# hassony2/homan

Measured on AMD Instinct MI355X. Metric: optimisation iters/sec (30-frame 256^2 clip), higher is better.
Workload: dtype f32

## Files before the change

### homan_amd/csrc/raster_lines.hip

```cpp
#include "raster_ws.h"

__global__ __launch_bounds__(256) void k_bwd_masks(const float* __restrict__ gin, int mode,
                                                   const float* __restrict__ upstream,
                                                   const float* __restrict__ keep_sum, int B, int S,
                                                   const unsigned short* __restrict__ alpha16,
                                                   float* __restrict__ gimg, unsigned short* __restrict__ planes,
                                                   int clip_len)
{
    if (mode == 1 && upstream[0] > 0.0f) return;
    const int w = threadIdx.x >> 6, lane = threadIdx.x & 63;
    const int is = 2 * S, tiles_x = S / HM_TILE, ntiles = tiles_x * tiles_x;
    const int tile = blockIdx.x * 4 + w, b = blockIdx.y;
    if (tile >= ntiles) return;
    const int ty = tile / tiles_x, tx = tile % tiles_x;
    const int rr = lane >> 3, cc = lane & 7;
    const int r = ty * HM_TILE + rr, c = tx * HM_TILE + cc;
    const long po = ((long)b * S + r) * S + c;
    unsigned long long cq[4];
#pragma unroll
    for (int dy = 0; dy < 2; ++dy) {
        const unsigned aw = alpha16[(((long)b * (is / 16) + ty) * (is / 16) + tx) * 16 + 2 * rr + dy];
#pragma unroll
        for (int dx = 0; dx < 2; ++dx) cq[2 * dy + dx] = __ballot((aw >> (2 * cc + dx)) & 1u);
    }
    unsigned long long nq[4], pq[4];
    if (mode == 3) {
#pragma unroll
        for (int dy = 0; dy < 2; ++dy) {
            const long at = ((long)b * is + 2 * r + dy) * is + 2 * c;
            const float2 g2 = *reinterpret_cast<const float2*>(gin + at);
            *reinterpret_cast<float2*>(gimg + at) = g2;
            nq[2 * dy] = __ballot(g2.x < 0.0f); pq[2 * dy] = __ballot(g2.x > 0.0f);
            nq[2 * dy + 1] = __ballot(g2.y < 0.0f); pq[2 * dy + 1] = __ballot(g2.y > 0.0f);
        }
    } else {
        float g = gin[po];
        if (mode == 1) {
            float s = upstream[0] * 2.0f;
            g = s * g / keep_sum[b / clip_len] / (float)clip_len;
        }
        gimg[po] = g;
        const unsigned long long nb1 = __ballot(g < 0.0f), pb1 = __ballot(g > 0.0f);
#pragma unroll
        for (int k = 0; k < 4; ++k) { nq[k] = nb1; pq[k] = pb1; }
    }
    const Ballots4 cov = {cq[0], cq[1], cq[2], cq[3]}, nbv = {nq[0], nq[1], nq[2], nq[3]}, pbv = {pq[0], pq[1], pq[2], pq[3]};
    emit_planes(cov, nbv, pbv, b, B, is, tx, ty, lane, planes);
}


__device__ __forceinline__ int sweep_family(float a0, float a1, int is, int& d0_from)
{
    d0_from = 0;
    if (!(a0 != a1)) return 0;
    d0_from = (int)fmaxf(ceilf(fminf(a0, a1)), 0.0f);
    const int d0_to = (int)fminf(fmaxf(a0, a1), (float)is - 1.0f);
    return max(0, d0_to - d0_from + 1);
}

__device__ __forceinline__ int sweep_face_record(long bf, const float* __restrict__ faces9, const FaceBox* __restrict__ boxes,
                                                 const unsigned char* __restrict__ owned, int F, int is, SweepFace& rec)
{
    const int b = (int)(bf / F), fi = (int)(bf - (long)b * F);
    const unsigned mask = (reinterpret_cast<const uint2*>(boxes)[bf].x >> 14) & 3u;
    const unsigned char own0 = owned[(long)b * 2 * F + fi], own1 = owned[(long)b * 2 * F + F + fi];
    const float* src = faces9 + bf * 9;
    float sx[3], sy[3];
#pragma unroll
    for (int k = 0; k < 3; ++k) { sx[k] = src[3 * k]; sy[k] = src[3 * k + 1]; }
    const bool act0 = (mask & 1u) && own0;
    const bool act1 = (mask & 2u) && own1;
    if (!(act0 || act1)) return 0;
#pragma unroll
    for (int k = 0; k < 3; ++k) { rec.px[k] = topix(sx[k], is); rec.py[k] = topix(sy[k], is); }
    int n = 0;
#pragma unroll
    for (int var = 0; var < 2; ++var)
#pragma unroll
        for (int e = 0; e < 3; ++e)
#pragma unroll
            for (int axis = 0; axis < 2; ++axis) {
                const int k0 = e, k1 = (e + 1) % 3;
                const int v0 = var ? 2 - k0 : k0, v1 = var ? 2 - k1 : k1;
                int from;
                const int c = sweep_family(axis ? rec.py[v0] : rec.px[v0], axis ? rec.py[v1] : rec.px[v1], is, from);
                if (var ? act1 : act0) n += c;
                rec.cum[var * 6 + e * 2 + axis] = (unsigned short)n;
            }
    rec.bf = (int)bf;
    rec.b = b;
    return n;
}

__device__ __forceinline__ void sweep_compact(int blk, int nblk, int fpt, const float* __restrict__ faces9,
                                              const FaceBox* __restrict__ boxes, const unsigned char* __restrict__ owned,
                                              int B, int F, int is, double* __restrict__ parts, const SweepList& sl,
                                              int clip_len)
{
    __shared__ int s_wsum[4][2];
    __shared__ unsigned long long s_base;
    const int tid = threadIdx.x, lane = tid & 63, wv = tid >> 6;
    const int per_clip = nblk / (B / clip_len), clip = blk / per_clip;
    const long cbase = (long)clip * clip_len * F;
    const long bf0 = cbase + ((long)(blk - clip * per_clip) * 256 + tid) * fpt, nbf = cbase + (long)clip_len * F;
    int nk[4], n = 0, hasf = 0;
#pragma unroll
    for (int k = 0; k < 4; ++k) {
        SweepFace rec;
        nk[k] = (k < fpt && bf0 + k < nbf) ? sweep_face_record(bf0 + k, faces9, boxes, owned, F, is, rec) : 0;
        n += nk[k];
        hasf += nk[k] > 0 ? 1 : 0;
    }
    const int inc_i = hm_wave_scan_incl(n), inc_f = hm_wave_scan_incl(hasf);
    if (lane == 63) { s_wsum[wv][0] = inc_i; s_wsum[wv][1] = inc_f; }
    __syncthreads();
    int pre_i = 0, pre_f = 0, tot_i = 0, tot_f = 0;
#pragma unroll
    for (int k = 0; k < 4; ++k) {
        if (k < wv) { pre_i += s_wsum[k][0]; pre_f += s_wsum[k][1]; }
        tot_i += s_wsum[k][0];
        tot_f += s_wsum[k][1];
    }
    if (tid == 0)
        s_base = tot_f ? atomicAdd(sl.cnt, ((unsigned long long)tot_f << 32) | (unsigned)((tot_i + SWEEP_UNIT - 1) & ~(SWEEP_UNIT - 1))) : 0ull;
    __syncthreads();
    const unsigned long long base = s_base;
    int off = (int)(base & 0xffffffffull) + pre_i + inc_i - n;
    int idx = (int)(base >> 32) + pre_f + inc_f - hasf;
#pragma unroll
    for (int k = 0; k < 4; ++k) {
        const long bf = bf0 + k;
        if (k >= fpt || bf >= nbf) break;
        bool zero = nk[k] == 0;
        if (nk[k] > 0) {
            SweepFace rec;
            const int nn = sweep_face_record(bf, faces9, boxes, owned, F, is, rec);
            const int u_lo = off >> SWEEP_USHIFT, u_hi = (off + nn - 1) >> SWEEP_USHIFT;
            const bool over = u_hi >= sl.ucap || u_hi + idx >= sl.slot_cap;
            rec.off = off;
            rec.flags = over ? 1 : 0;
            zero = u_hi > u_lo;
            const uint4* r4 = reinterpret_cast<const uint4*>(&rec);
            uint4* t4 = reinterpret_cast<uint4*>(sl.tab + idx);
#pragma unroll
            for (int q = 0; q < 4; ++q) t4[q] = r4[q];
            sl.offs[idx] = off;
            for (int u = (off + SWEEP_UNIT - 1) >> SWEEP_USHIFT; (u << SWEEP_USHIFT) < off + nn && u < sl.ucap; ++u)
                sl.ufirst[u] = (unsigned)idx;
            off += nn;
            ++idx;
        }
        if (zero) {
            double* o = parts + bf * 6;
#pragma unroll
            for (int q = 0; q < 6; ++q) o[q] = 0.0;
        }
    }
    if (tid == 0) {
        const unsigned int t = atomicAdd(sl.done, 1u);
        if (t == (unsigned)nblk - 1u) {
            sl.total[0] = atomicExch(sl.cnt, 0ull);
            atomicExch(sl.done, 0u);
        }
    }
}


#ifndef LINES_NL
#define LINES_NL 2
#endif
#ifdef LINES_REVERSED
#define LINES_BLK(i, n) ((n) - 1 - (i))
#else
#define LINES_BLK(i, n) (i)
#endif
template <bool W32>
__global__ __launch_bounds__(256) void k_bwd_lines(const unsigned short* __restrict__ planes,
                                                   const float* __restrict__ gimg, const float* __restrict__ dimg,
                                                   int mode, const float* __restrict__ upstream,
                                                   const float* __restrict__ keep_sum,
                                                   const int* __restrict__ idx_map, int B, int S,
                                                   SweepSrc* __restrict__ srcs, uint4* __restrict__ lrec,
                                                   int ncomp, int fpt, const float* __restrict__ faces9,
                                                   const FaceBox* __restrict__ boxes,
                                                   const unsigned char* __restrict__ owned, int F,
                                                   double* __restrict__ parts, SweepList sl, int clip_len,
                                                   unsigned short* __restrict__ lsum, int nred,
                                                   const float* __restrict__ red_partials, float* __restrict__ frame_rec,
                                                   float* __restrict__ loss_out, int out_stride,
                                                   const unsigned int* __restrict__ ts_flag,
                                                   unsigned long long* __restrict__ ts_slots)
{
    HM_CHAIN_KERNEL();
    const unsigned long long ts_t0 = (unsigned long long)wall_clock64();
    const bool ts_on = hm_ts_enabled(ts_flag) && threadIdx.x == 0;
    if (ts_on) hm_ts_store(ts_slots, blockIdx.x, 0, ts_t0);
    const int blk = (int)blockIdx.x;
    __shared__ unsigned long long s_w[16][LINES_NL][SWEEP_CUMW];
    __shared__ int s_ex[16][LINES_NL][SWEEP_CUMW];
    if (blk < ncomp) {
        sweep_compact(blk, ncomp, fpt, faces9, boxes, owned, B, F, 2 * S, parts, sl, clip_len);
        if (ts_on) hm_ts_store(ts_slots, blockIdx.x, 1, (unsigned long long)wall_clock64());
        return;
    }
    if (blk < ncomp + nred) {
        sil_reduce_frame(blk - ncomp, red_partials, (S / 8) * (S / 8), keep_sum, frame_rec, loss_out, nullptr, clip_len,
                         out_stride);
        if (ts_on) hm_ts_store(ts_slots, blockIdx.x, 1, (unsigned long long)wall_clock64());
        return;
    }
    typedef typename HmOff<W32>::t OFF;
    const int l = threadIdx.x & 15, grp = threadIdx.x >> 4;
    const bool ts_row = l == 0 && hm_ts_enabled(ts_flag);
    const int is = 2 * S, wpl = is / 64, T = is / 16;
    const unsigned Lw = (unsigned)(LINES_BLK(blk - ncomp - nred, (int)gridDim.x - ncomp - nred)) * (16u * LINES_NL);
    const bool valid = Lw < 4u * (unsigned)B * (unsigned)is;
    const unsigned fr = Lw / (unsigned)is;
    const int d00 = (int)(Lw - fr * (unsigned)is) + grp * LINES_NL, b = (int)(fr % (unsigned)B), pa = (int)(fr / (unsigned)B);
    const OFF L0 = (OFF)Lw + (OFF)(grp * LINES_NL);
    const int axis = pa & 1, pl = pa >> 1;
    unsigned long long mine[LINES_NL];
#pragma unroll
    for (int j = 0; j < LINES_NL; ++j) mine[j] = 0ull;
    if (valid && l < wpl) {
        unsigned long long raw[4];
#pragma unroll
        for (int jj = 0; jj < 4; ++jj) {
            OFF at;
            if (axis) {
                const int t = is - 1 - d00 - (LINES_NL - 1);
                at = ((((OFF)b * T + (t >> 4)) * T + (4 * l + jj)) * 4 + pl) * 16 + (t & 15);
            } else {
                at = ((((OFF)b * T + (T - 1 - (4 * l + jj))) * T + (d00 >> 4)) * 4 + (2 + pl)) * 16 + (d00 & 15);
            }
#if LINES_NL == 4
            raw[jj] = *reinterpret_cast<const unsigned long long*>(hm_at<W32>(planes, at));
#elif LINES_NL == 2
            raw[jj] = *reinterpret_cast<const unsigned int*>(hm_at<W32>(planes, at));
#else
            raw[jj] = *hm_at<W32>(planes, at);
#endif
        }
#pragma unroll
        for (int j = 0; j < LINES_NL; ++j) {
            const int sel = axis ? LINES_NL - 1 - j : j;
#pragma unroll
            for (int jj = 0; jj < 4; ++jj) mine[j] |= ((raw[jj] >> (16 * sel)) & 0xffffull) << (16 * jj);
        }
    }
    bool any = false;
#pragma unroll
    for (int j = 0; j < LINES_NL; ++j) {
        const OFF L = L0 + j;
        const int d0 = d00 + j;
        const int c = __popcll(mine[j]);
        int incl = c;
        incl += __builtin_amdgcn_update_dpp(0, incl, 0x111, 0xf, 0xf, false);
        incl += __builtin_amdgcn_update_dpp(0, incl, 0x112, 0xf, 0xf, false);
        incl += __builtin_amdgcn_update_dpp(0, incl, 0x114, 0xf, 0xf, false);
        incl += __builtin_amdgcn_update_dpp(0, incl, 0x118, 0xf, 0xf, false);
        const int excl = incl - c;
        if (valid && l < wpl) *hm_at<W32>(lrec, L * wpl + l) = make_uint4((unsigned)mine[j], (unsigned)(mine[j] >> 32), (unsigned)excl, 0u);
        int lo = mine[j] ? 64 * l + __builtin_ctzll(mine[j]) : 0xffff, hi = mine[j] ? 64 * l + 64 - __builtin_clzll(mine[j]) : 0;
        lo = min(lo, __builtin_amdgcn_update_dpp(0xffff, lo, 0x111, 0xf, 0xf, false)); hi = max(hi, __builtin_amdgcn_update_dpp(0, hi, 0x111, 0xf, 0xf, false));
        lo = min(lo, __builtin_amdgcn_update_dpp(0xffff, lo, 0x112, 0xf, 0xf, false)); hi = max(hi, __builtin_amdgcn_update_dpp(0, hi, 0x112, 0xf, 0xf, false));
        lo = min(lo, __builtin_amdgcn_update_dpp(0xffff, lo, 0x114, 0xf, 0xf, false)); hi = max(hi, __builtin_amdgcn_update_dpp(0, hi, 0x114, 0xf, 0xf, false));
        lo = min(lo, __builtin_amdgcn_update_dpp(0xffff, lo, 0x118, 0xf, 0xf, false)); hi = max(hi, __builtin_amdgcn_update_dpp(0, hi, 0x118, 0xf, 0xf, false));
        const unsigned wm = (unsigned)(__ballot(mine[j] != 0ull) >> (16 * (grp & 3))) & 0xffffu;
        if (valid && l == 15)
            *reinterpret_cast<uint2*>(hm_at<W32>(lsum, ((((OFF)b * 2 + axis) * is + d0) * 2 + pl) * 4)) =
                make_uint2((unsigned)lo | ((unsigned)hi << 16), wm);
        any = any || wm != 0u;
        s_w[grp][j][l] = mine[j];
        s_ex[grp][j][l] = excl;
    }
    wave_sync();
    if (!valid || !any) {
        if (ts_row) atomicMax(ts_slots + 2 * blockIdx.x + 1, (unsigned long long)wall_clock64());
        return;
    }
    const bool from_dimg = mode == 2 || (mode == 1 && upstream[0] > 0.0f);
    const float* gi = (from_dimg ? dimg : gimg) + (long)b * S * S;
    const float gs = from_dimg ? upstream[0] * 2.0f : 0.f, ks = from_dimg ? keep_sum[b / clip_len] : 1.f;
    const float up4 = (mode == 4 || mode == 5) ? upstream[b] * 2.0f : 0.f;
    const int* idx = idx_map + (long)b * is * is;
    const float* gfull = gimg + (long)b * is * is;
#pragma unroll 1
    for (int j = 0; j < LINES_NL; ++j) {
        const int d0 = d00 + j;
        const OFF out0 = (L0 + j) * is;
        for (int k = 0; k < wpl; ++k) {
            const unsigned long long w = s_w[grp][j][k];
            if (w == 0ull) continue;
            const int base = s_ex[grp][j][k];
            float gl[4];
            int ow[4];
#pragma unroll
            for (int q = 0; q < 4; ++q) {
                const int pos = 16 * q + l;
                gl[q] = 0.f;
                ow[q] = -1;
                if (!((w >> pos) & 1ull)) continue;
                const int d1 = (k << 6) + pos;
                const int xi = axis ? d1 : d0, yi = axis ? d0 : d1;
                if (mode == 5) gl[q] = pl ? 1.0f : -1.0f;
                else if (mode == 3 || mode == 4) gl[q] = gfull[(is - 1 - yi) * is + xi];
                else gl[q] = gi[((is - 1 - yi) >> 1) * S + (xi >> 1)];
                if (pl) ow[q] = idx[yi * is + xi];
            }
#pragma unroll
            for (int q = 0; q < 4; ++q) {
                const int pos = 16 * q + l;
                if (!((w >> pos) & 1ull)) continue;
                SweepSrc r;
                r.d1 = (k << 6) + pos;
                float g = gl[q];
                if (mode == 4 || mode == 5) g = up4 * g;
                else if (mode != 3) {
                    if (from_dimg) g = gs * g / ks / (float)clip_len;
                    g = 0.25f * g;
                }
                r.g = g;
                r.owner = ow[q];
                *hm_at<W32>(srcs, out0 + (OFF)(base + __popcll(w & ((1ull << pos) - 1ull)))) = r;
            }
        }
    }
    if (ts_row) atomicMax(ts_slots + 2 * blockIdx.x + 1, (unsigned long long)wall_clock64());
}

void hm_launch_bwd_masks(const SilWs& w, const float* gin, int mode, const float* upstream, const float* keep_sum, int B, int S,
                         int clip_len, hipStream_t stream)
{
    const int ntiles = (S / 8) * (S / 8);
    hipLaunchKernelGGL(k_bwd_masks, dim3(hm_cdiv(ntiles, 4), B), dim3(256), 0, stream, gin, mode, upstream, keep_sum, B, S,
                       w.alpha16, w.gimg, w.planes, clip_len);
}
void hm_launch_lines(const SilWs& w, int B, int F, int S, int mode, const float* upstream, const float* keep_sum, int clip_len,
                     hipStream_t stream, float* loss_out, int out_stride)
{
    const int nred = loss_out ? B : 0;
    const int fpt = (long)clip_len * F >= 400000 ? 4 : 1;
    const int ncomp = (B / clip_len) * hm_cdiv((long)clip_len * F, 256 * fpt);
    const bool w32 = hm_offsets_fit_32(B, S);
    hipLaunchKernelGGL(w32 ? k_bwd_lines<true> : k_bwd_lines<false>, dim3(ncomp + nred + hm_cdiv(4L * B * 2 * S, 16 * LINES_NL)), dim3(256), 0, stream, w.planes,
                       w.gimg, w.dimg, mode, upstream, keep_sum, w.idx_map, B, S, w.srcs, w.lrec, ncomp, fpt, w.faces9, w.boxes,
                       w.owned, F, w.parts, w.sweep, clip_len, w.lsum, nred, w.partials, w.frame_rec, loss_out, out_stride,
                       w.counter + 24, w.ts + 2 * ts_raster_units(B, S));
}
```

Before: 6627.

## Load-balance line emission via shared task list and interleaved row mapping

Each block now gathers every non-empty (row, line, word) segment into a shared-memory task list, built with a wave ballot and prefix popcounts. All 16 groups then pull tasks from that list round-robin, so lines with dense coverage no longer serialise on the group that owns them. Lines per group rise from 2 to 4, and rows are interleaved across blocks so that dense regions spread over more blocks. The cost is a block-wide __syncthreads and extra shared memory, and the grid shrinks, which may reduce occupancy.

```diff
diff --git a/homan_amd/csrc/raster_lines.hip b/homan_amd/csrc/raster_lines.hip
--- a/homan_amd/csrc/raster_lines.hip
+++ b/homan_amd/csrc/raster_lines.hip
@@ -167,13 +167,20 @@
 
 
 #ifndef LINES_NL
-#define LINES_NL 2
+#define LINES_NL 4
 #endif
 #ifdef LINES_REVERSED
 #define LINES_BLK(i, n) ((n) - 1 - (i))
 #else
 #define LINES_BLK(i, n) (i)
 #endif
+#ifndef LINES_IL
+#define LINES_IL 4
+#endif
+__device__ __forceinline__ int lines_row_d0(int g, int G, int row)
+{
+    return ((g + (row / LINES_IL) * G) * LINES_IL + row % LINES_IL) * LINES_NL;
+}
 template <bool W32>
 __global__ __launch_bounds__(256) void k_bwd_lines(const unsigned short* __restrict__ planes,
                                                    const float* __restrict__ gimg, const float* __restrict__ dimg,
@@ -198,6 +205,8 @@
     const int blk = (int)blockIdx.x;
     __shared__ unsigned long long s_w[16][LINES_NL][SWEEP_CUMW];
     __shared__ int s_ex[16][LINES_NL][SWEEP_CUMW];
+    __shared__ unsigned short s_task[4][4 * LINES_NL * SWEEP_CUMW];
+    __shared__ int s_nt[4];
     if (blk < ncomp) {
         sweep_compact(blk, ncomp, fpt, faces9, boxes, owned, B, F, 2 * S, parts, sl, clip_len);
         if (ts_on) hm_ts_store(ts_slots, blockIdx.x, 1, (unsigned long long)wall_clock64());
@@ -213,11 +222,14 @@
     const int l = threadIdx.x & 15, grp = threadIdx.x >> 4;
     const bool ts_row = l == 0 && hm_ts_enabled(ts_flag);
     const int is = 2 * S, wpl = is / 64, T = is / 16;
-    const unsigned Lw = (unsigned)(LINES_BLK(blk - ncomp - nred, (int)gridDim.x - ncomp - nred)) * (16u * LINES_NL);
-    const bool valid = Lw < 4u * (unsigned)B * (unsigned)is;
-    const unsigned fr = Lw / (unsigned)is;
-    const int d00 = (int)(Lw - fr * (unsigned)is) + grp * LINES_NL, b = (int)(fr % (unsigned)B), pa = (int)(fr / (unsigned)B);
-    const OFF L0 = (OFF)Lw + (OFF)(grp * LINES_NL);
+    const unsigned wi = (unsigned)(LINES_BLK(blk - ncomp - nred, (int)gridDim.x - ncomp - nred));
+    const int G = is / (16 * LINES_NL);
+    const unsigned fr = wi / (unsigned)G;
+    const int sg = (int)(wi - fr * (unsigned)G);
+    const bool valid = fr < 4u * (unsigned)B;
+    const int d00 = lines_row_d0(sg, G, grp), b = (int)(fr % (unsigned)B), pa = (int)(fr / (unsigned)B);
+    const OFF Ls = (OFF)fr * (OFF)is;
+    const OFF L0 = Ls + (OFF)d00;
     const int axis = pa & 1, pl = pa >> 1;
     unsigned long long mine[LINES_NL];
 #pragma unroll
@@ -248,7 +260,8 @@
             for (int jj = 0; jj < 4; ++jj) mine[j] |= ((raw[jj] >> (16 * sel)) & 0xffffull) << (16 * jj);
         }
     }
-    bool any = false;
+    const int wv = threadIdx.x >> 6, lane = threadIdx.x & 63;
+    int nt = 0;
 #pragma unroll
     for (int j = 0; j < LINES_NL; ++j) {
         const OFF L = L0 + j;
@@ -266,16 +279,20 @@
         lo = min(lo, __builtin_amdgcn_update_dpp(0xffff, lo, 0x112, 0xf, 0xf, false)); hi = max(hi, __builtin_amdgcn_update_dpp(0, hi, 0x112, 0xf, 0xf, false));
         lo = min(lo, __builtin_amdgcn_update_dpp(0xffff, lo, 0x114, 0xf, 0xf, false)); hi = max(hi, __builtin_amdgcn_update_dpp(0, hi, 0x114, 0xf, 0xf, false));
         lo = min(lo, __builtin_amdgcn_update_dpp(0xffff, lo, 0x118, 0xf, 0xf, false)); hi = max(hi, __builtin_amdgcn_update_dpp(0, hi, 0x118, 0xf, 0xf, false));
-        const unsigned wm = (unsigned)(__ballot(mine[j] != 0ull) >> (16 * (grp & 3))) & 0xffffu;
+        const unsigned long long bal = __ballot(mine[j] != 0ull);
+        const unsigned wm = (unsigned)(bal >> (16 * (grp & 3))) & 0xffffu;
         if (valid && l == 15)
             *reinterpret_cast<uint2*>(hm_at<W32>(lsum, ((((OFF)b * 2 + axis) * is + d0) * 2 + pl) * 4)) =
                 make_uint2((unsigned)lo | ((unsigned)hi << 16), wm);
-        any = any || wm != 0u;
         s_w[grp][j][l] = mine[j];
         s_ex[grp][j][l] = excl;
-    }
-    wave_sync();
-    if (!valid || !any) {
+        if (mine[j] != 0ull) s_task[wv][nt + __popcll(bal & ((1ull << lane) - 1ull))] = (unsigned short)((grp << 6) | (j << 4) | l);
+        nt += __popcll(bal);
+    }
+    if (lane == 0) s_nt[wv] = nt;
+    __syncthreads();
+    const int n1 = s_nt[0], n2 = n1 + s_nt[1], n3 = n2 + s_nt[2], ntot = n3 + s_nt[3];
+    if (grp >= ntot) {
         if (ts_row) atomicMax(ts_slots + 2 * blockIdx.x + 1, (unsigned long long)wall_clock64());
         return;
     }
@@ -286,44 +303,44 @@
     const int* idx = idx_map + (long)b * is * is;
     const float* gfull = gimg + (long)b * is * is;
 #pragma unroll 1
-    for (int j = 0; j < LINES_NL; ++j) {
-        const int d0 = d00 + j;
-        const OFF out0 = (L0 + j) * is;
-        for (int k = 0; k < wpl; ++k) {
-            const unsigned long long w = s_w[grp][j][k];
-            if (w == 0ull) continue;
-            const int base = s_ex[grp][j][k];
-            float gl[4];
-            int ow[4];
-#pragma unroll
-            for (int q = 0; q < 4; ++q) {
-                const int pos = 16 * q + l;
-                gl[q] = 0.f;
-                ow[q] = -1;
-                if (!((w >> pos) & 1ull)) continue;
-                const int d1 = (k << 6) + pos;
-                const int xi = axis ? d1 : d0, yi = axis ? d0 : d1;
-                if (mode == 5) gl[q] = pl ? 1.0f : -1.0f;
-                else if (mode == 3 || mode == 4) gl[q] = gfull[(is - 1 - yi) * is + xi];
-                else gl[q] = gi[((is - 1 - yi) >> 1) * S + (xi >> 1)];
-                if (pl) ow[q] = idx[yi * is + xi];
+    for (int t = grp; t < ntot; t += 16) {
+        const int seg = (t >= n1 ? 1 : 0) + (t >= n2 ? 1 : 0) + (t >= n3 ? 1 : 0);
+        const unsigned code = s_task[seg][t - (seg == 0 ? 0 : seg == 1 ? n1 : seg == 2 ? n2 : n3)];
+        const int tr = (int)(code >> 6), j = (int)(code >> 4) & 3, k = (int)code & 15;
+        const int d0 = lines_row_d0(sg, G, tr) + j;
+        const OFF out0 = (Ls + (OFF)d0) * is;
+        const unsigned long long w = s_w[tr][j][k];
+        const int base = s_ex[tr][j][k];
+        float gl[4];
+        int ow[4];
+#pragma unroll
+        for (int q = 0; q < 4; ++q) {
+            const int pos = 16 * q + l;
+            gl[q] = 0.f;
+            ow[q] = -1;
+            if (!((w >> pos) & 1ull)) continue;
+            const int d1 = (k << 6) + pos;
+            const int xi = axis ? d1 : d0, yi = axis ? d0 : d1;
+            if (mode == 5) gl[q] = pl ? 1.0f : -1.0f;
+            else if (mode == 3 || mode == 4) gl[q] = gfull[(is - 1 - yi) * is + xi];
+            else gl[q] = gi[((is - 1 - yi) >> 1) * S + (xi >> 1)];
+            if (pl) ow[q] = idx[yi * is + xi];
+        }
+#pragma unroll
+        for (int q = 0; q < 4; ++q) {
+            const int pos = 16 * q + l;
+            if (!((w >> pos) & 1ull)) continue;
+            SweepSrc r;
+            r.d1 = (k << 6) + pos;
+            float g = gl[q];
+            if (mode == 4 || mode == 5) g = up4 * g;
+            else if (mode != 3) {
+                if (from_dimg) g = gs * g / ks / (float)clip_len;
+                g = 0.25f * g;
             }
-#pragma unroll
-            for (int q = 0; q < 4; ++q) {
-                const int pos = 16 * q + l;
-                if (!((w >> pos) & 1ull)) continue;
-                SweepSrc r;
-                r.d1 = (k << 6) + pos;
-                float g = gl[q];
-                if (mode == 4 || mode == 5) g = up4 * g;
-                else if (mode != 3) {
-                    if (from_dimg) g = gs * g / ks / (float)clip_len;
-                    g = 0.25f * g;
-                }
-                r.g = g;
-                r.owner = ow[q];
-                *hm_at<W32>(srcs, out0 + (OFF)(base + __popcll(w & ((1ull << pos) - 1ull)))) = r;
-            }
+            r.g = g;
+            r.owner = ow[q];
+            *hm_at<W32>(srcs, out0 + (OFF)(base + __popcll(w & ((1ull << pos) - 1ull)))) = r;
         }
     }
     if (ts_row) atomicMax(ts_slots + 2 * blockIdx.x + 1, (unsigned long long)wall_clock64());
```

New measurement: 6687, median of 6. Within noise of the previous version (+0.9%).
